# hila-chefer/Transformer-Explainability

Measured on AMD Instinct MI355X. Metric: relevance maps/sec (ViT-B/16 224^2, batch 64 per GPU, generate_LRP transformer_attribution), higher is better.
Workload: dtype f32 (3xbf16 split operands, 6 products, fp32 accumulate)

## Files before the change

### include/te_relprop.h

```cpp
#ifndef TE_RELPROP_H
#define TE_RELPROP_H

#include <stddef.h>
#include <stdint.h>

#ifdef __cplusplus
extern "C" {
#endif

typedef void* te_stream_t;
typedef uint16_t te_bf16_t;

enum {
  TE_OK = 0,
  TE_ERR_INVALID_ARG = -1,
  TE_ERR_WORKSPACE = -2,
  TE_ERR_UNSUPPORTED = -3,
  TE_ERR_NO_DEVICE = -4
};

enum { TE_VARIANT_OURS = 0, TE_VARIANT_LRP = 1, TE_IMPL_SIMPLE = 0x100 };

enum { TE_ROLLOUT_NORMALISE = 1, TE_ROLLOUT_CLS_FIXUP = 2, TE_ROLLOUT_ROW0 = 4 };

// ... 109 lines not shown
int te_gradcam_headmean_f32(const float* grad, const float* cam, float* out,
                            int64_t B, int64_t H, int64_t N, te_stream_t stream);

size_t te_rollout_workspace_bytes(int64_t L, int64_t B, int64_t N);
size_t te_rollout_row0_workspace_bytes(int64_t B, int64_t N);
int te_rollout_f32(const float* cams, int64_t L, int64_t start_layer, int64_t B, int64_t N,
                   int flags, float* joint, void* ws, size_t ws_bytes, te_stream_t stream);

#define TE_X6_TILE_AUTO 0
#define TE_X6_TILE_128 1
#define TE_X6_TILE_256 2
#define TE_X6_TILE_128x128 3
#define TE_X6_TEST_DROP_HANDOVER 0x200
#define TE_X6_WHOLE_TILES 0x10000
#define TE_X6_TEST_SMALL_GRID 0x4000
#define TE_X6_TILE_Z_SHIFT 10
#define TE_X6_TILE_C_SHIFT 12
#define TE_X6_PHASE_SPLIT 4
#define TE_X6_PHASE_Z 8
#define TE_X6_PHASE_C 16
#define TE_X6_PHASE_MASK 28
int te_linear_relprop_x6_supported(int64_t T, int64_t in_f, int64_t out_f);
size_t te_linear_relprop_x6_workspace_bytes(int64_t T, int64_t in_f, int64_t out_f);
size_t te_linear_x6_weight_planes_bytes(int64_t in_f, int64_t out_f);
size_t te_linear_x6_planes_bytes(int64_t rows, int64_t K);
int te_linear_x6_prepare_weights_f32(const float* W, int64_t in_f, int64_t out_f, void* planes, size_t planes_bytes,
                                     te_stream_t stream);
int te_linear_x6_split_abs_f32(const float* X, int64_t rows, int64_t K, void* planes, size_t planes_bytes,
                               te_stream_t stream);
int te_linear_relprop_x6_f32(const float* R, const float* r_scale, int64_t r_scale_stride, int64_t rows_per_sample,
// ... 301 lines not shown
```

### transformer-explainability_amd/csrc/te_api.hip

```cpp
#include "te_common.h"

#include <string.h>

extern "C" int te_version(void) { return 705;  }

#ifndef TE_BUILD_ID
#define TE_BUILD_ID "unstamped"
#endif
extern "C" const char* te_build_id(void) { return TE_BUILD_ID; }

extern "C" const char* te_status_string(int status) {
  switch (status) {
    case TE_OK: return "ok";
    case TE_ERR_INVALID_ARG: return "invalid argument";
    case TE_ERR_WORKSPACE: return "workspace missing, misaligned or too small";
    case TE_ERR_UNSUPPORTED: return "shape not supported by the gfx950 kernels";
    case TE_ERR_NO_DEVICE: return "no gfx950 device visible";
    default: break;
  }
  if (status > 0) return hipGetErrorString((hipError_t)status);
  return "unknown status";
}

extern "C" int te_device_check(void) {
// ... 10 lines not shown
```

### transformer-explainability_amd/csrc/te_linear_x6.hip

```cpp
#include <algorithm>
#include <cmath>
#include <type_traits>

#include "te_x6.h"

namespace {

constexpr int kRB = 3 * kFrag;
constexpr int kMinFrag = 4;
constexpr float kCancelTol = 0.0078125f;
constexpr int kSpinMillis = 250;
constexpr int kErrWord = 1023;


enum { MODE_Z = 0, MODE_C = 1, MODE_G = 2, MODE_ZI = 3, MODE_Z1 = 4, MODE_CI = 5, MODE_X = 6 };

__device__ __forceinline__ float bf16_f32(unsigned b) { return __uint_as_float(b << 16); }

enum { OP_ABS = 0, OP_POS = 1, OP_NEG = 2, OP_ID = 3 };
template <int OP>
__device__ __forceinline__ float apply_op(float x) {
  if constexpr (OP == OP_ID) return x;
  if constexpr (OP == OP_ABS) return __int_as_float(__float_as_int(x) & 0x7fffffff);
  const int b = __float_as_int(x);
  if constexpr (OP == OP_POS) return __int_as_float(b > 0 ? b : 0);
  return __int_as_float(b < 0 ? b : 0);
}

template <int OP, bool TRANSPOSE>
__global__ __launch_bounds__(256) void split_kernel(const float* __restrict__ src, unsigned char* __restrict__ dst,
// ... 104 lines not shown
  unsigned p[8][3];
#pragma unroll
  for (int e = 0; e < 8; ++e) split3_pk(v[2 * e], v[2 * e + 1], p[e]);
  auto store = [&](unsigned char* d) __attribute__((always_inline)) {
#pragma unroll
    for (int q = 0; q < 3; ++q)
#pragma unroll
      for (int kh = 0; kh < 2; ++kh) {
        u32x4 w;
#pragma unroll
        for (int e = 0; e < 4; ++e) w[e] = p[4 * kh + e][q];
        *reinterpret_cast<u32x4*>(d + q * kFrag + kh * 512) = w;
      }
  };
  store(dst + ((rb * nks + ks) * 3) * kFrag + r * 16);
  if constexpr (SRC == SRC_GELU_FWD) {
#pragma unroll
    for (int e = 0; e < 8; ++e) {
      const unsigned m = p[e][0] & 0x80008000u;
      p[e][0] &= 0x7fff7fffu;
      p[e][1] ^= m & (((p[e][1] & 0x7fff7fffu) + 0x7fff7fffu) & 0x80008000u);
      p[e][2] ^= m & (((p[e][2] & 0x7fff7fffu) + 0x7fff7fffu) & 0x80008000u);
    }
    store(dst_abs + ((rb * nks + ks) * 3) * kFrag + r * 16);
  }
}

__global__ __launch_bounds__(256) void zero_words_kernel(u32x4* __restrict__ p) {
  p[(size_t)blockIdx.x * 256 + threadIdx.x] = u32x4{0u, 0u, 0u, 0u};
}

// ... 67 lines not shown

constexpr int kStages = 2;
template <int WM>
struct X6Geo {
  static constexpr int NWM = (WM == 1) ? 1 : 2, NWN = (WM == 0) ? 2 : 4, MI = (WM == 0) ? 2 : 4;
  static constexpr int NW = NWM * NWN, THREADS = 64 * NW, WPS = (WM == 0) ? 3 : 2;
  static constexpr int TM = NWM * MI * 32, TT = NWN * 64;
  static constexpr int NPA = 3 * NWM * MI, NPB = 3 * NWN * 2;
  static constexpr int ACC = MI * 2 * 16;
  static constexpr int MAX_SPX = (WM == 2) ? 32 : (WM == 1) ? 64 : 96;
};

template <int WM, int MODE>
struct X6Lds {
  using GEO = X6Geo<WM>;
  static constexpr bool STAGED = (MODE == MODE_Z || MODE == MODE_ZI || MODE == MODE_Z1) && GEO::MI == 4;
  static constexpr int STAGES = kStages * (GEO::NPA + GEO::NPB) * kFrag;
  static constexpr int MAIN = (STAGED && GEO::NW * 16384 > STAGES) ? GEO::NW * 16384 : STAGES;
  static constexpr int TOTAL = MAIN + GEO::NW * 512 + 16;
};

template <int WM, int MODE>
__global__ __launch_bounds__(X6Geo<WM>::THREADS, X6Geo<WM>::WPS) void x6_kernel(const X6Params p) {
  using GEO = X6Geo<WM>;
  constexpr int NW = GEO::NW, NWM = GEO::NWM, NWN = GEO::NWN, MI = GEO::MI;
  constexpr bool IS_Z = (MODE == MODE_Z || MODE == MODE_ZI || MODE == MODE_Z1);
  constexpr bool IS_C = (MODE == MODE_C || MODE == MODE_CI);
  constexpr int G = IS_C ? 6 : 3;
  constexpr int NPA = GEO::NPA, NPB = GEO::NPB;
  constexpr int NP = NPA + NPB;
  static_assert(NPA / 3 == NW, "each wave stages one weight-side block");
  constexpr int PBW = NPB / 3 / NW;
  constexpr int STAGE = NP * kFrag;
  constexpr int GROUPS = NPA / G;
  constexpr int LDS_MAIN = X6Lds<WM, MODE>::MAIN;
  extern __shared__ __attribute__((aligned(16))) unsigned char smem[];

  const int lane = threadIdx.x & 63;
  const int wave = __builtin_amdgcn_readfirstlane(threadIdx.x >> 6);
  const int wm = wave / NWN, wn = wave % NWN;
  const int lane16 = lane * 16;
// ... 43 lines not shown
    }

    const unsigned char* srcA;
    if constexpr (!IS_C)
      srcA = p.A + (int64_t)(tm * GROUPS + wave) * p.a_group_stride + (int64_t)k0 * kRB;
    else
      srcA = p.A + (int64_t)(tm * GROUPS + (wave >> 1)) * p.a_group_stride + (int64_t)k0 * (2 * kRB) + (wave & 1) * kRB;
    const unsigned char* srcB[PBW];
#pragma unroll
    for (int u = 0; u < PBW; ++u) {
      const int cb = min(tn * (GEO::TT / 32) + wave * PBW + u, p.ncb - 1);
      srcB[u] = p.B + (int64_t)cb * p.b_rb_stride + (int64_t)k0 * kRB;
    }
    unsigned char* const ldsA = smem + wave * kRB;
    unsigned char* const ldsB = smem + NPA * kFrag + wave * (PBW * kRB);
    auto stage_in = [&](int stg, int adv) __attribute__((always_inline)) {
      srcA += adv * (G * kFrag);
#pragma unroll
      for (int u = 0; u < PBW; ++u) srcB[u] += adv * kRB;
#pragma unroll
      for (int q = 0; q < 3; ++q) glds16(srcA + q * kFrag + lane16, ldsA + stg * STAGE + q * kFrag);
#pragma unroll
      for (int u = 0; u < PBW; ++u)
#pragma unroll
        for (int q = 0; q < 3; ++q) glds16(srcB[u] + q * kFrag + lane16, ldsB + stg * STAGE + (u * 3 + q) * kFrag);
    };

    auto wait_for = [&](unsigned* flag) -> bool {
      unsigned* const ok_word = reinterpret_cast<unsigned*>(smem + LDS_MAIN + NW * 512);
      if (threadIdx.x == 0) {
        unsigned spins = 0, ok = 1u;
        const long long t_begin = wall_clock64();
        while (__hip_atomic_load(flag, __ATOMIC_RELAXED, __HIP_MEMORY_SCOPE_AGENT) == 0u) {
          __builtin_amdgcn_s_sleep(8);
          if ((++spins & 63u) == 0u &&
              (__hip_atomic_load(p.status, __ATOMIC_RELAXED, __HIP_MEMORY_SCOPE_AGENT) != 0u ||
               wall_clock64() - t_begin > p.spin_ticks)) {
            ok = 0u;
            break;
          }
// ... 24 lines not shown
            for (int e = 0; e < 4; ++e) acc[mi][ni][4 * c + e] = handed_over ? v[e] : __builtin_nanf("");
          }
          ip += 4 * 64;
          asm volatile("" : "+v"(ip));
        }
    } else {
#pragma unroll
      for (int mi = 0; mi < MI; ++mi)
#pragma unroll
        for (int ni = 0; ni < 2; ++ni)
#pragma unroll
          for (int e = 0; e < 16; ++e) acc[mi][ni][e] = 0.0f;
    }

    stage_in(0, 0);
    int st = 0;
    bf16x8 a[MI][3], b[2][3];
    for (int ks = k0; ks < k1; ++ks) {
      asm volatile("s_waitcnt vmcnt(0) lgkmcnt(0)" ::: "memory");
      __builtin_amdgcn_s_barrier();
      const unsigned char* sA = smem + st * STAGE + wm * (MI * kRB) + lane16;
      const unsigned char* sB = smem + st * STAGE + NPA * kFrag + wn * (2 * kRB) + lane16;
      const unsigned aA = (unsigned)(uintptr_t)sA, aB = (unsigned)(uintptr_t)sB;
#define X6_SB __builtin_amdgcn_sched_barrier(0)
#define X6_RDB(ni, r) \
  asm volatile("ds_read_b128 %0, %1 offset:%2" : "=v"(b[ni][PB[r]]) : "v"(aB), "i"((ni) * kRB + PB[r] * kFrag))
#define X6_RDA(mi, r) \
  asm volatile("ds_read_b128 %0, %1 offset:%2" : "=v"(a[mi][PA[r]]) : "v"(aA), "i"((mi) * kRB + PA[r] * kFrag))
#define X6_WAIT(n)                                                           \
  X6_SB;                                                                     \
// ... 50 lines not shown
      X6_SB;
#pragma unroll
      for (int q6 = 3; q6 < 6; ++q6) {
        X6_MM(0, 0, q6); X6_MM(1, 0, q6); X6_MM(1, 1, q6); X6_MM(0, 1, q6);
        X6_MM(2, 1, q6); X6_MM(2, 0, q6); X6_MM(3, 0, q6); X6_MM(3, 1, q6);
        X6_SB;
      }
      }
#undef X6_SB
#undef X6_RDB
#undef X6_RDA
#undef X6_WAIT
#undef X6_MM
#undef X6_RD_HEAD
#undef X6_RD_TAIL
      st = (st + 1 == kStages) ? 0 : st + 1;
    }

    auto publish = [&](float* dst, unsigned* flag) __attribute__((always_inline)) {
      f32x4* op = reinterpret_cast<f32x4*>(dst) + (size_t)wave * (GEO::ACC / 4) * 64 + lane;
#pragma unroll
      for (int mi = 0; mi < MI; ++mi)
#pragma unroll
        for (int ni = 0; ni < 2; ++ni) {
#pragma unroll
          for (int c = 0; c < 4; ++c) {
            f32x4 v;
#pragma unroll
            for (int e = 0; e < 4; ++e) v[e] = acc[mi][ni][4 * c + e];
            op[c * 64] = v;
          }
          op += 4 * 64;
// ... 73 lines not shown
          for (int g = 0; g < 4; ++g) {
            asm volatile("ds_read_b128 %0, %1 offset:%2" : "=v"(r4[g]) : "v"(rda[g]), "i"(buf * 8192));
            if constexpr (MODE != MODE_Z1)
              asm volatile("ds_read_b128 %0, %1 offset:%2" : "=v"(y4[g]) : "v"(rda[g]), "i"(buf * 8192 + 4096));
            asm volatile("ds_read_b128 %0, %1 offset:%2" : "=v"(b4[g]) : "v"(bia), "i"((mi * 32 + 8 * g) * 4));
          }
          asm volatile("s_waitcnt lgkmcnt(0)" ::: "memory");
          if (bi + 2 < 2 * MI) request(bi + 2, buf);
          X6_PASS4(r4[0], r4[1], r4[2], r4[3]);
          if constexpr (MODE != MODE_Z1) X6_PASS4(y4[0], y4[1], y4[2], y4[3]);
          X6_PASS4(b4[0], b4[1], b4[2], b4[3]);
          unsigned w[4][3][2];
          unsigned long long any_cancel = 0;
          auto z_of = [&](int g, int c0, f32x2& z2, f32x2& a2) __attribute__((always_inline)) {
            a2 = f32x2{acc[mi][ni][4 * g + c0], acc[mi][ni][4 * g + c0 + 1]};
            if constexpr (MODE == MODE_Z)
              z2 = f32x2{0.5f, 0.5f} * ((f32x2{y4[g][c0], y4[g][c0 + 1]} - f32x2{b4[g][c0], b4[g][c0 + 1]}) + a2);
            else if constexpr (MODE == MODE_ZI)
              z2 = f32x2{0.5f, 0.5f} * ((f32x2{y4[g][c0], y4[g][c0 + 1]} - f32x2{b4[g][c0], b4[g][c0 + 1]}) - a2);
            else
              z2 = a2;
          };
          auto cancels = [&](float z, float a_abs) __attribute__((always_inline)) -> bool {
            if constexpr (MODE == MODE_Z) return !(z > kCancelTol * a_abs);
            else if constexpr (MODE == MODE_ZI) return !(-z > kCancelTol * a_abs);
            else return false;
          };
#pragma unroll
          for (int g = 0; g < 4; ++g) {
            float sv4[4];
#pragma unroll
            for (int c0 = 0; c0 < 4; c0 += 2) {
              f32x2 z2, a2;
              z_of(g, c0, z2, a2);
              f32x2 rr = {r4[g][c0], r4[g][c0 + 1]};
              if (p.rs) rr = rr * f32x2{f[ni], f[ni]};
              const f32x2 sv = sd2(rr, z2);
#pragma unroll
              for (int e = 0; e < 2; ++e) {
// ... 87 lines not shown
          if (bi + 1 < 2 * MI) load_block(bi + 1, buf ^ 1);
        } else {
          load_block(bi, 0);
        }
        unsigned w[4][3][2];
        unsigned bad = 0;
#pragma unroll
        for (int g = 0; g < 4; ++g) {
          const f32x4 b4 = *reinterpret_cast<const f32x4*>(bias_lds + mi * 32 + 8 * g + 4 * h);
          float sv4[4];
#pragma unroll
          for (int c = 0; c < 4; ++c) {
            const float a_abs = acc[mi][ni][4 * g + c];
            float z;
            bool cancel;
            if constexpr (MODE == MODE_Z) {
              z = 0.5f * ((y4[buf][g][c] - b4[c]) + a_abs);
              cancel = !(z > kCancelTol * a_abs);
            } else if constexpr (MODE == MODE_ZI) {
              z = 0.5f * ((y4[buf][g][c] - b4[c]) - a_abs);
              cancel = !(-z > kCancelTol * a_abs);
            } else {
              z = a_abs;
              cancel = false;
            }
            bad |= (cancel ? 1u : 0u) << (4 * g + c);
            float rr = r4[buf][g][c];
            if (p.rs) rr = rr * f[ni];
            float sv = te_sd(rr, z);
            asm volatile("" : "+v"(sv));
            sv4[c] = (live[ni] && !cancel) ? sv : 0.0f;
// ... 180 lines not shown
inline X6Workspace general_workspace(int64_t T, int64_t in_f, int64_t out_f) { return x6_workspace(T, in_f, out_f, 2, 2, kGeneralPasses); }

struct X6WeightPlanes { size_t c, total; };
inline X6WeightPlanes weight_planes(int64_t in_f, int64_t out_f) {
  const size_t c = te_align_up(planes_bytes(out_f, in_f), 256);
  return {c, c + te_align_up(2 * planes_bytes(in_f, out_f), 256)};
}
struct X6WeightPlanesLrp { size_t wn, wpT, wnT, total; };
inline X6WeightPlanesLrp weight_planes_lrp(int64_t in_f, int64_t out_f) {
  const size_t za = te_align_up(planes_bytes(out_f, in_f), 256), ca = te_align_up(planes_bytes(in_f, out_f), 256);
  return {za, 2 * za, 2 * za + ca, 2 * za + 2 * ca};
}

constexpr int kTileMask = TE_X6_TILE_128 | TE_X6_TILE_256 | TE_X6_TILE_128x128;
constexpr int kProductFlags = kTileMask | TE_X6_WHOLE_TILES | TE_X6_TEST_DROP_HANDOVER | TE_X6_TEST_SMALL_GRID;
constexpr int kRuleFlags = kProductFlags | TE_X6_PHASE_MASK | (kTileMask << TE_X6_TILE_Z_SHIFT) | (kTileMask << TE_X6_TILE_C_SHIFT);

inline int pick_wm(int64_t in_f, int64_t out_f) {
  if (out_f % 256 == 0 && in_f % 128 == 0) return 2;
  if (out_f % 128 == 0 && in_f % 64 == 0) return 1;
  return 0;
}

inline long long spin_ticks_for_current_device() {
  static long long cached[64] = {};
  int dev = 0;
  if (hipGetDevice(&dev) != hipSuccess || dev < 0 || dev >= 64) dev = 0;
  if (cached[dev] == 0) {
    int khz = 0;
    if (hipDeviceGetAttribute(&khz, hipDeviceAttributeWallClockRate, dev) != hipSuccess || khz <= 0) khz = 100000;
    cached[dev] = (long long)khz * kSpinMillis;
// ... 166 lines not shown
  return TE_OK;
}

extern "C" int te_gelu_backward_x6_planes_f32(const float* dy, const float* x, int64_t rows, int64_t K, void* planes,
                                              size_t planes_bytes_, te_stream_t stream_) {
  const int rc = check_producer(dy && x && planes, te_aligned16(dy) && te_aligned16(x), te_aligned16(planes), rows, K, planes_bytes_);
  if (rc != TE_OK) return rc;
  gelu_split_lds_kernel<SRC_GELU_BWD><<<producer_grid(rows, K), dim3(256), 0, (hipStream_t)stream_>>>(
      dy, x, nullptr, (unsigned char*)planes, nullptr, rows, K);
  TE_RETURN_IF_LAUNCH_FAILED();
  return TE_OK;
}

extern "C" int te_gelu_forward_x6_planes_f32(const float* x, float* y, int64_t rows, int64_t K, void* planes, void* planes_abs,
                                             size_t planes_bytes_, te_stream_t stream_) {
  const int rc = check_producer(x && y && planes && planes_abs, te_aligned16(x) && te_aligned16(y),
                                te_aligned16(planes) && te_aligned16(planes_abs), rows, K, planes_bytes_);
  if (rc != TE_OK) return rc;
  gelu_split_lds_kernel<SRC_GELU_FWD><<<producer_grid(rows, K), dim3(256), 0, (hipStream_t)stream_>>>(
      nullptr, x, y, (unsigned char*)planes, (unsigned char*)planes_abs, rows, K);
  TE_RETURN_IF_LAUNCH_FAILED();
  return TE_OK;
}

extern "C" size_t te_gemm_x6_workspace_bytes(int64_t T, int64_t K, int64_t M) {
  return te_gemm_x6_supported(T, K, M) ? gemm_workspace(T, K, M).total : 0;
}

extern "C" int te_gemm_x6_f32(const float* X, const void* x_planes, const void* w_planes, const float* bias, float* out,
                              int64_t T, int64_t K, int64_t M, int flags, unsigned* status, void* ws, size_t ws_bytes,
                              te_stream_t stream_) {
  if ((!X && !x_planes) || !w_planes || !out) return TE_ERR_INVALID_ARG;
// ... 32 lines not shown
  if (!te_linear_relprop_x6_supported(T, in_f, out_f)) return TE_ERR_UNSUPPORTED;
  if (!ws || ws_bytes < te_linear_relprop_x6_workspace_bytes(T, in_f, out_f) || !te_aligned16(ws)) return TE_ERR_WORKSPACE;
  if (!te_aligned16(X) || !te_aligned16(W) || !te_aligned16(R) || !te_aligned16(Y) || !te_aligned16(out) ||
      !te_aligned16(w_planes) || (bias && !te_aligned16(bias)) || (x_planes && !te_aligned16(x_planes)))
    return TE_ERR_UNSUPPORTED;
  if (bad_r_scale(r_scale, rows_per_sample, T)) return TE_ERR_INVALID_ARG;
  if ((flags & ~kRuleFlags) != 0) return TE_ERR_INVALID_ARG;
  const int phases = (flags & TE_X6_PHASE_MASK) ? (flags & TE_X6_PHASE_MASK) : TE_X6_PHASE_MASK;
  hipStream_t stream = (hipStream_t)stream_;
  const X6Workspace l = rule_workspace(T, in_f, out_f);
  unsigned char* Ss = l.sp(ws, 0);
  const unsigned char* wz = (const unsigned char*)w_planes;
  const unsigned char* wc = wz + weight_planes(in_f, out_f).c;

  if (phases & TE_X6_PHASE_SPLIT) zero_flag_regions(l.flag_region(ws, 0), kRulePasses, stream);
  if (!x_planes) {
    if (phases & TE_X6_PHASE_SPLIT) {
      int rc = te_linear_x6_split_abs_f32(X, T, in_f, l.x(ws, 0), planes_bytes(T, in_f), stream_);
      if (rc != TE_OK) return rc;
    }
    x_planes = l.x(ws, 0);
  }
  const int wm_max = pick_wm(in_f, out_f);
  const int pz = (flags >> TE_X6_TILE_Z_SHIFT) & kTileMask, pc = (flags >> TE_X6_TILE_C_SHIFT) & kTileMask;
  const int wm_z = choose_geo(wm_max, T, out_f, pz ? pz : (flags & kTileMask), 256, true);
  const int wm_c = choose_geo(wm_max, T, 2 * in_f, pc ? pc : (flags & kTileMask));
  const X6Params p = rule_params(call_params(T, l.acc(ws), bias, out, status, flags), R, r_scale, r_scale_stride, rows_per_sample,
                                 X, W, Y);
  int rc;
  if (phases & TE_X6_PHASE_Z) {
    rc = launch_pass<MODE_Z>(p, wm_z, wz, (const unsigned char*)x_planes, Ss, in_f, out_f, l.flag_region(ws, 0), stream, 1.0f);
    if (rc != TE_OK) return rc;
  }
  if (phases & TE_X6_PHASE_C) {
    rc = launch_pass<MODE_C>(p, wm_c, wc, Ss, Ss, in_f, out_f, l.flag_region(ws, 1), stream, 1.0f);
    if (rc != TE_OK) return rc;
  }
  TE_RETURN_IF_LAUNCH_FAILED();
  return TE_OK;
}

extern "C" int te_linear_relprop_x6_general_supported(int64_t T, int64_t in_f, int64_t out_f, int variant) {
  if (!te_linear_relprop_x6_supported(T, in_f, out_f)) return 0;
  if (variant == TE_VARIANT_LRP) return (in_f % 128 == 0) ? 1 : 0;
  return variant == TE_VARIANT_OURS ? 1 : 0;
}
// ... 123 lines not shown
```

### transformer-explainability_amd/ops.py

```python
from __future__ import annotations

import contextlib
import os
from typing import Optional, Sequence, Tuple

import torch

from . import _lib
from ._lib import (TE_HEADMEAN_CLAMP, TE_HEADMEAN_ROW0, TE_IMPL_SIMPLE, TE_RATIONALE_CLAMP, TE_ROLLOUT_CLS_FIXUP,
                   TE_ROLLOUT_NORMALISE, TE_ROLLOUT_ROW0, TE_VARIANT_LRP, TE_VARIANT_OURS)
from ._lib import (TE_X6_PHASE_C, TE_X6_PHASE_SPLIT, TE_X6_PHASE_Z, TE_X6_TEST_DROP_HANDOVER,
                   TE_X6_TEST_SMALL_GRID, TE_X6_TILE_C_SHIFT, TE_X6_TILE_Z_SHIFT, TE_X6_WHOLE_TILES)

Tensor = torch.Tensor
_VARIANTS = {"ours": TE_VARIANT_OURS, "lrp": TE_VARIANT_LRP}

FORCE_SIMPLE = False
KERNEL_TIMER = None
_NULL = contextlib.nullcontext()


def _timed(name: str, flops: float = 0.0, nbytes: float = 0.0):
    return _NULL if KERNEL_TIMER is None else KERNEL_TIMER(name, float(flops), float(nbytes))


class Deferred:
    __slots__ = ("t", "scale")
# ... 265 lines not shown
    out_f, in_f = W.shape
    dims = (in_f, out_f) if transposed else (out_f, in_f)
    return _cached_planes(W, cache, "x6_gemm_planes_T" if transposed else "x6_gemm_planes", lambda Wd: (_prepare_planes(
        _c(Wd), "te_linear_x6_planes_bytes", "te_linear_x6_split_matrix_f32", dims, int(transposed)),))[0]


def linear_relprop_x6_supported(T: int, in_f: int, out_f: int) -> bool:
    return bool(_lib.load().te_linear_relprop_x6_supported(int(T), int(in_f), int(out_f)))


def gemm_x6_supported(T: int, K: int, M: int) -> bool:
    return bool(_lib.load().te_gemm_x6_supported(int(T), int(K), int(M)))


X6_KEEP_ABS = os.environ.get("TE_X6_KEEP_ABS", "1") not in ("", "0")


def _x_abs_key(X: Tensor, T: int, K: int):
    return (X.data_ptr(), X._version, T, K, str(X.device))


def post_x_planes(cache: dict, X: Tensor, xs: Tensor, xa: Tensor):
    K = X.shape[-1]
    cache["x_planes_from_producer"] = (_x_abs_key(X, X.numel() // K, K), xs, xa, X)


def take_x_planes(cache: dict, X: Tensor, T: int, K: int):
    hit = cache.pop("x_planes_from_producer", None)
    if hit is not None and hit[0] == _x_abs_key(X, T, K) and hit[3].data_ptr() == X.data_ptr():
        return hit[1], hit[2]
    return None


def drop_x_planes(cache: dict, with_abs: bool = False):
    cache.pop("x_planes_from_producer", None)
    if with_abs:
        cache.pop("x_abs_planes", None)
# ... 52 lines not shown
    K = X.shape[-1]
    lead = X.shape[:-1]
    T = X.numel() // K
    Xc = None if x_planes is not None else _c(X).reshape(-1, K)
    like = X if Xc is None else Xc
    out = torch.empty((T, M), dtype=torch.float32, device=X.device)
    bc = None if bias is None else _c(bias.detach())
    with _on_device(like) as lib:
        ws = _ws(lib.te_gemm_x6_workspace_bytes(T, K, M), like)
        x_bytes = (6.0 if x_planes is not None else 10.0) * T * K
        xs = x_planes
        if xs is None and keep_abs is not None:
            got = take_x_planes(keep_abs, X, T, K)
            if got is not None:
                xs, x_bytes = got[0], 6.0 * T * K
                post_x_abs_planes(keep_abs, X, T, K, got[1])
        if xs is not None and xs.numel() * xs.element_size() < lib.te_linear_x6_planes_bytes(T, K):
            raise _lib.TeError(f"gemm_x6: the operand planes handed in hold {xs.numel() * xs.element_size()} bytes, "
                               f"[{T}, {K}] needs {lib.te_linear_x6_planes_bytes(T, K)}")
        with _timed(timer_name, 12.0 * T * K * M, x_bytes + 6.0 * K * M + 4.0 * T * M):
            if xs is None and keep_abs is not None and rule_takes_abs_planes(T, K, M):
                nb = lib.te_linear_x6_planes_bytes(T, K)
                xs, xa = _ws(nb, Xc), _ws(nb, Xc)
                _lib.check(lib.te_linear_x6_split_dual_f32(_ptr(Xc), T, K, _ptr(xs), _ptr(xa), nb, _stream(Xc)),
                           "te_linear_x6_split_dual_f32")
                post_x_abs_planes(keep_abs, X, T, K, xa)
            _lib.check(lib.te_gemm_x6_f32(_ptr(Xc) if Xc is not None else None, _ptr(xs), _ptr(w_planes), _ptr(bc), _ptr(out),
                                          T, K, M, (X6_TILE | X6_FLAGS) & ~0x3c00, _ptr(x6_status(X.device)), _ptr(ws),
                                          ws.numel(), _stream(like)), "te_gemm_x6_f32")
    return out.reshape(*lead, M)


def linear_relprop(R: Tensor, X: Tensor, W: Tensor, alpha: float = 1.0, variant="ours",
                   Y: Optional[Tensor] = None, bias: Optional[Tensor] = None, cache: Optional[dict] = None) -> Tensor:
    if _any_f64(R, X, W):
        return linear_relprop_f64(R, X, W, alpha=alpha, variant=variant)
    if _is_bf16(X) or _is_bf16(W):
        return linear_relprop_bf16(R, X, W, alpha=alpha, variant=variant, cache=cache)
    out_f, in_f = W.shape
    lead = X.shape[:-1]
    R, r_scale = _split_deferred(R)
# ... 15 lines not shown
    var_code = var & 0xff
    general = (USE_LINEAR_X6 and not (var & TE_IMPL_SIMPLE) and not (var_code == TE_VARIANT_OURS and alpha == 1)
               and all(t.data_ptr() % 16 == 0 for t in (Rc, Xc, Wc))
               and (var_code == TE_VARIANT_LRP or (USE_FORWARD_OUTPUT and Y is not None))
               and bool(_lib.load().te_linear_relprop_x6_general_supported(T, in_f, out_f, var_code)))
    if general:
        Yg = bg = None
        if var_code == TE_VARIANT_OURS:
            Yg = _c(Y.detach()).reshape(-1, out_f)
            bg = None if bias is None else _c(bias.detach())
            general = Yg.shape[0] == T and Yg.data_ptr() % 16 == 0 and (bg is None or bg.data_ptr() % 16 == 0)
    if general:
        wp = x6_weight_planes(W, cache) if var_code == TE_VARIANT_OURS else None
        wpl = x6_weight_planes_lrp(W, cache) if var_code == TE_VARIANT_LRP else None
        xa = take_x_abs_planes(cache, X, T, in_f) if cache is not None and var_code == TE_VARIANT_OURS else None
        gemm = 2.0 * T * in_f * out_f
        halves = 2 if alpha != 1 else 1
        units = (18.0 if var_code == TE_VARIANT_OURS else 24.0) * halves
        with _on_device(Xc) as lib, _timed("linear_x6_general", units * gemm,
                                           halves * (6.0 * (2 * T * in_f + 3 * in_f * out_f + 2 * T * out_f) + 16.0 * T * in_f)):
            ws = _ws(lib.te_linear_relprop_x6_general_workspace_bytes(T, in_f, out_f, var_code), Xc)
            _lib.check(lib.te_linear_relprop_x6_general_f32(_ptr(Rc), rs_ptr, rs_stride, rps, _ptr(Xc), _ptr(Wc), _ptr(wp),
                                                            _ptr(wpl), _ptr(xa), _ptr(Yg), _ptr(bg), _ptr(out), T, in_f,
                                                            out_f, float(alpha), var_code, (X6_TILE | X6_FLAGS) & ~0x3c00,
                                                            _ptr(x6_status(Xc.device)), _ptr(ws), ws.numel(), _stream(Xc)),
                       "te_linear_relprop_x6_general_f32")
            if X6_CHECK:
                x6_raise_if_failed(Xc.device)
        return out.reshape(*lead, in_f)
    if fwd:
        Yc = _c(Y.detach()).reshape(-1, out_f)
        bc = None if bias is None else _c(bias.detach())
        if Yc.shape[0] != T:
            raise _lib.TeError(f"Linear.relprop: Y has {Yc.shape[0]} rows, X has {T}")
    if (fwd and USE_LINEAR_X6 and Yc.data_ptr() % 16 == 0 and (bc is None or bc.data_ptr() % 16 == 0)
            and _lib.load().te_linear_relprop_x6_supported(T, in_f, out_f)):
        planes = x6_weight_planes(W, cache)
        xa = take_x_abs_planes(cache, X, T, in_f) if cache is not None else None
        with _on_device(Xc) as lib:
            ws = _ws(lib.te_linear_relprop_x6_workspace_bytes(T, in_f, out_f), Xc)
            status = x6_status(Xc.device)

            def call(flags):
                _lib.check(lib.te_linear_relprop_x6_f32(_ptr(Rc), rs_ptr, rs_stride, rps, _ptr(Xc), _ptr(Wc), _ptr(planes),
                                                        _ptr(xa), _ptr(Yc), _ptr(bc), _ptr(out), T, in_f, out_f,
                                                        X6_TILE | X6_FLAGS | flags, _ptr(status), _ptr(ws), ws.numel(),
                                                        _stream(Xc)),
                           "te_linear_relprop_x6_f32")
            if KERNEL_TIMER is None:
                call(0)
            else:
                gemm = 2.0 * T * in_f * out_f
                if xa is None:
                    with _timed("linear_x6_split", 0.0, 10.0 * T * in_f):
                        call(TE_X6_PHASE_SPLIT)
                else:
                    call(TE_X6_PHASE_SPLIT)
                with _timed("linear_x6_zpass", 6.0 * gemm, 6.0 * (T * in_f + in_f * out_f + T * out_f) + 8.0 * T * out_f):
                    call(TE_X6_PHASE_Z)
                with _timed("linear_x6_cpass", 12.0 * gemm, 6.0 * (T * out_f + 2 * in_f * out_f) + 8.0 * T * in_f):
                    call(TE_X6_PHASE_C)
# ... 242 lines not shown
        _lib.check(lib.te_attention_backward_strided_f32(_ptr(d_out), N * C, 64, C, _ptr(q), qb, qh, qn, _ptr(k), kb, kh, kn,
                                                         _ptr(v), vb, vh, vn, _ptr(attn), _ptr(d_attn), _ptr(dq), dqb, dqh,
                                                         dqn, _ptr(dk), dkb, dkh, dkn, _ptr(dv), dvb, dvh, dvn, B, H, N, D,
                                                         float(scale), int(bool(need_qk)), _ptr(ws), ws.numel(),
                                                         _stream(d_out)), "te_attention_backward_strided_f32")
    return d_attn


def attention_forward_planes_supported(qkv: Tensor, num_heads: int) -> bool:
    B, N, C3 = qkv.shape
    C = C3 // 3
    return (qkv.is_cuda and qkv.dtype == torch.float32 and C % num_heads == 0 and C // num_heads == 64 and N <= 224
            and bool(_lib.load().te_attention_forward_supported(N, 64)))


def attention_forward(qkv: Tensor, num_heads: int, scale: float, planes: bool = False):
    if _is_bf16(qkv):
        if planes:
            raise _lib.TeError("attention_forward(planes=True): operand planes are emitted from float32 activations only")
        qkv = _c16(qkv)
        C = qkv.shape[-1] // 3
        out, attn, zqk, _ = attention_forward_qkv_bf16(qkv[..., :C], qkv[..., C:2 * C], qkv[..., 2 * C:], num_heads, scale)
        return out, attn, zqk
    qkv = _c(qkv)
    B, N, C3 = qkv.shape
    C = C3 // 3
    H, D = num_heads, C // num_heads
    if not _lib.load().te_attention_forward_supported(N, D):
        if planes:
            raise _lib.TeError("attention_forward(planes=True): shape not served by te_attention_forward_planes_f32")
        out, attn, zqk, _ = attention_forward_qkv(qkv[..., :C], qkv[..., C:2 * C], qkv[..., 2 * C:], num_heads, scale)
        return out, attn, zqk
    out = torch.empty((B, N, C), dtype=torch.float32, device=qkv.device)
    attn = torch.empty((B, H, N, N), dtype=torch.float32, device=qkv.device)
    zqk = torch.empty((B, H, N, N), dtype=torch.float32, device=qkv.device)
    extra = 12.0 * B * N * C if planes else 0.0
    with _on_device(qkv) as lib, _timed("attention_forward", 4.0 * B * H * N * N * D, 4.0 * B * (2 * H * N * N + 4 * N * C) + extra):
        if planes:
            nb = lib.te_linear_x6_planes_bytes(B * N, C)
            xs, xa = _ws(nb, qkv), _ws(nb, qkv)
            _lib.check(lib.te_attention_forward_planes_f32(_ptr(qkv), _ptr(zqk), _ptr(attn), _ptr(out), _ptr(xs), _ptr(xa), nb,
                                                           B, H, N, D, float(scale), _stream(qkv)),
                       "te_attention_forward_planes_f32")
            return out, attn, zqk, xs, xa
        _lib.check(lib.te_attention_forward_f32(_ptr(qkv), _ptr(zqk), _ptr(attn), _ptr(out), B, H, N, D, float(scale),
                                                _stream(qkv)), "te_attention_forward_f32")
    return out, attn, zqk


def attention_backward(d_out: Tensor, qkv: Tensor, attn: Tensor, num_heads: int, scale: float,
                       need_qk: bool = True, out: Optional[Tensor] = None) -> Tuple[Tensor, Optional[Tensor]]:
    if _is_bf16(d_out) or _is_bf16(qkv) or _is_bf16(attn):
        qkv = _c16(qkv)
        C = qkv.shape[-1] // 3
        d_qkv = torch.empty_like(qkv)
# ... 79 lines not shown
        return self

    def __exit__(self, *exc):
        global _GELU_BWD_HANDOFF
        _GELU_BWD_HANDOFF -= 1


def gelu_backward_handoff_active() -> bool:
    return _GELU_BWD_HANDOFF > 0


def gelu_planes_supported(x: Tensor) -> bool:
    return bool(X6_FUSE_GELU and x.dim() >= 2 and x.shape[-1] >= 16 and x.shape[-1] % 16 == 0)


def gelu_forward_planes(x: Tensor):
    x = _c(x)
    K = x.shape[-1]
    T = x.numel() // K
    y = torch.empty_like(x)
    with _on_device(x) as lib, _timed("gelu_forward", 0.0, (4.0 * 2 + 12.0) * x.numel()):
        nb = lib.te_linear_x6_planes_bytes(T, K)
        xs, xa = _ws(nb, x), _ws(nb, x)
        _lib.check(lib.te_gelu_forward_x6_planes_f32(_ptr(x), _ptr(y), T, K, _ptr(xs), _ptr(xa), nb, _stream(x)),
                   "te_gelu_forward_x6_planes_f32")
    return y, xs, xa


def gelu_backward_planes(dy: Tensor, x: Tensor) -> Tensor:
    dy, x = _c(dy), _c(x)
    K = x.shape[-1]
    T = x.numel() // K
    with _on_device(x) as lib, _timed("gelu_backward", 0.0, (4.0 * 2 + 6.0) * x.numel()):
        nb = lib.te_linear_x6_planes_bytes(T, K)
        planes = _ws(nb, x)
        _lib.check(lib.te_gelu_backward_x6_planes_f32(_ptr(dy), _ptr(x), T, K, _ptr(planes), nb, _stream(x)),
                   "te_gelu_backward_x6_planes_f32")
    return planes
# ... 1313 lines not shown
```

### transformer-explainability_amd/producers.py

```python
from __future__ import annotations

import torch

from . import ops


def usable(x: torch.Tensor) -> bool:
    return ops.USE_FUSED_PRODUCERS and torch.is_tensor(x) and ops.layernorm_supported(x)


def gelu_usable(x: torch.Tensor) -> bool:
    return (ops.USE_FUSED_PRODUCERS and torch.is_tensor(x) and x.is_cuda and x.dtype == torch.float32
            and x.numel() > 0 and x.numel() % 4 == 0)


def norm_usable(x: torch.Tensor, norm) -> bool:
    return (usable(x) and not norm.training and getattr(norm, "weight", None) is not None
            and tuple(norm.normalized_shape) == (x.shape[-1],))


class _LayerNorm(torch.autograd.Function):
    @staticmethod
    def forward(ctx, x, weight, bias, eps):
        y, mean, rstd = ops.layernorm_forward(x, weight, bias, eps)
# ... 17 lines not shown
    @staticmethod
    def backward(ctx, d_bypass, dy):
        x, weight, mean, rstd = ctx.saved_tensors
        if dy is None:
            return d_bypass, None, None, None
        return ops.layernorm_backward(dy, x, weight, mean, rstd, add=d_bypass), None, None, None


class _Gelu(torch.autograd.Function):

    @staticmethod
    def forward(ctx, x, feeds, source):
        ctx.save_for_backward(x)
        ctx.source = source
        if feeds is not None:
            y, xs, xa = ops.gelu_forward_planes(x)
            ops.post_x_planes(feeds, y, xs, xa)
            return y
        return ops.gelu_forward(x)

    @staticmethod
    def backward(ctx, dy):
        (x,) = ctx.saved_tensors
        if ctx.source is not None:
            return ops.post_dy_planes(ctx.source, ops.gelu_backward_planes(dy, x), x), None, None
        return ops.gelu_backward(dy, x), None, None


class _Linear(torch.autograd.Function):

    @staticmethod
# ... 64 lines not shown
```

### transformer-explainability_amd/vit.py

```python
from __future__ import annotations

import torch
import torch.nn as nn

from . import methods, ops, producers
from . import rules as R_ours

__all__ = ["VisionTransformer", "vit_base_patch16_224", "vit_large_patch16_224", "deit_base_patch16_224",
           "compute_rollout_attention", "make_vit_module"]


def compute_rollout_attention(all_layer_matrices, start_layer=0):
    return ops.rollout(torch.stack(list(all_layer_matrices), 0), start_layer=start_layer, normalise=False)


def tail_full(model, cam, **kwargs):
    cam, _ = model.add.relprop(cam, **kwargs)
    cam = model.patch_embed.relprop(cam[:, 1:], **kwargs)
    return cam.sum(dim=1)


def tail_rollout(model, start_layer=0):
    mats = [blk.attn.get_attn_cam().clamp(min=0).mean(dim=1) for blk in model.blocks]
    return compute_rollout_attention(mats, start_layer=start_layer)[:, 0, 1:]
# ... 62 lines not shown
                slot.zero_()
            else:
                slot.copy_(g)
        return grad.view(B, N, 3 * H * D), None


def split_qkv(qkv, num_heads):
    return _SplitQKV.apply(qkv, num_heads)


class _FusedAttention(torch.autograd.Function):

    @staticmethod
    def forward(ctx, qkv, num_heads, scale, module, feeds=None):
        if feeds is not None:
            out, attn, zqk, xs, xa = ops.attention_forward(qkv, num_heads, scale, planes=True)
            ops.post_x_planes(feeds, out, xs, xa)
        else:
            out, attn, zqk = ops.attention_forward(qkv, num_heads, scale)
        ctx.save_for_backward(qkv, attn, out)
        ctx.num_heads, ctx.scale, ctx.module = num_heads, scale, module
        ctx.mark_non_differentiable(attn, zqk)
        ctx.set_materialize_grads(False)
        return out, attn, zqk

    @staticmethod
    def backward(ctx, d_out, _d_attn_unused, _d_zqk_unused):
        qkv, attn, out = ctx.saved_tensors
        if d_out is None:
            return None, None, None, None, None
        stop = bool(getattr(ctx.module, "_fused_stop_backward", False))
# ... 363 lines not shown
```

Measured before the change: 1012.

## Reuse signed operand planes for relprop Z pass by taking abs on the fly

Producers (GELU, attention, forward GEMM split) no longer write a second set of absolute-value bf16 planes. The Z relevance pass gets a new signed mode that loads the signed X planes into registers, clears the sign of the high plane, flips the lower planes to match, and stores them to LDS itself instead of using direct global-to-LDS loads. This saves the extra plane writes and their memory footprint in the forward pass. In exchange the Z kernel does more register and ALU work and loses the asynchronous LDS load path, which could hurt its pipelining.

```diff
diff --git a/include/te_relprop.h b/include/te_relprop.h
--- a/include/te_relprop.h
+++ b/include/te_relprop.h
@@ -147,6 +147,7 @@
 #define TE_X6_TEST_DROP_HANDOVER 0x200
 #define TE_X6_WHOLE_TILES 0x10000
 #define TE_X6_TEST_SMALL_GRID 0x4000
+#define TE_X6_X_PLANES_SIGNED 0x20000
 #define TE_X6_TILE_Z_SHIFT 10
 #define TE_X6_TILE_C_SHIFT 12
 #define TE_X6_PHASE_SPLIT 4
diff --git a/transformer-explainability_amd/csrc/te_api.hip b/transformer-explainability_amd/csrc/te_api.hip
--- a/transformer-explainability_amd/csrc/te_api.hip
+++ b/transformer-explainability_amd/csrc/te_api.hip
@@ -2,7 +2,7 @@
 
 #include <string.h>
 
-extern "C" int te_version(void) { return 705;  }
+extern "C" int te_version(void) { return 706;  }
 
 #ifndef TE_BUILD_ID
 #define TE_BUILD_ID "unstamped"
diff --git a/transformer-explainability_amd/csrc/te_linear_x6.hip b/transformer-explainability_amd/csrc/te_linear_x6.hip
--- a/transformer-explainability_amd/csrc/te_linear_x6.hip
+++ b/transformer-explainability_amd/csrc/te_linear_x6.hip
@@ -13,7 +13,7 @@
 constexpr int kErrWord = 1023;
 
 
-enum { MODE_Z = 0, MODE_C = 1, MODE_G = 2, MODE_ZI = 3, MODE_Z1 = 4, MODE_CI = 5, MODE_X = 6 };
+enum { MODE_Z = 0, MODE_C = 1, MODE_G = 2, MODE_ZI = 3, MODE_Z1 = 4, MODE_CI = 5, MODE_X = 6, MODE_ZS = 7 };
 
 __device__ __forceinline__ float bf16_f32(unsigned b) { return __uint_as_float(b << 16); }
 
@@ -148,7 +148,7 @@
       }
   };
   store(dst + ((rb * nks + ks) * 3) * kFrag + r * 16);
-  if constexpr (SRC == SRC_GELU_FWD) {
+  if (SRC == SRC_GELU_FWD && dst_abs) {
 #pragma unroll
     for (int e = 0; e < 8; ++e) {
       const unsigned m = p[e][0] & 0x80008000u;
@@ -246,7 +246,7 @@
 template <int WM, int MODE>
 struct X6Lds {
   using GEO = X6Geo<WM>;
-  static constexpr bool STAGED = (MODE == MODE_Z || MODE == MODE_ZI || MODE == MODE_Z1) && GEO::MI == 4;
+  static constexpr bool STAGED = (MODE == MODE_Z || MODE == MODE_ZS || MODE == MODE_ZI || MODE == MODE_Z1) && GEO::MI == 4;
   static constexpr int STAGES = kStages * (GEO::NPA + GEO::NPB) * kFrag;
   static constexpr int MAIN = (STAGED && GEO::NW * 16384 > STAGES) ? GEO::NW * 16384 : STAGES;
   static constexpr int TOTAL = MAIN + GEO::NW * 512 + 16;
@@ -256,7 +256,9 @@
 __global__ __launch_bounds__(X6Geo<WM>::THREADS, X6Geo<WM>::WPS) void x6_kernel(const X6Params p) {
   using GEO = X6Geo<WM>;
   constexpr int NW = GEO::NW, NWM = GEO::NWM, NWN = GEO::NWN, MI = GEO::MI;
-  constexpr bool IS_Z = (MODE == MODE_Z || MODE == MODE_ZI || MODE == MODE_Z1);
+  constexpr bool SGN = MODE == MODE_ZS;
+  constexpr bool Z_ABS = MODE == MODE_Z || SGN;
+  constexpr bool IS_Z = (Z_ABS || MODE == MODE_ZI || MODE == MODE_Z1);
   constexpr bool IS_C = (MODE == MODE_C || MODE == MODE_CI);
   constexpr int G = IS_C ? 6 : 3;
   constexpr int NPA = GEO::NPA, NPB = GEO::NPB;
@@ -330,6 +332,7 @@
     }
     unsigned char* const ldsA = smem + wave * kRB;
     unsigned char* const ldsB = smem + NPA * kFrag + wave * (PBW * kRB);
+    u32x4 breg[SGN ? PBW : 1][3];
     auto stage_in = [&](int stg, int adv) __attribute__((always_inline)) {
       srcA += adv * (G * kFrag);
 #pragma unroll
@@ -339,7 +342,24 @@
 #pragma unroll
       for (int u = 0; u < PBW; ++u)
 #pragma unroll
-        for (int q = 0; q < 3; ++q) glds16(srcB[u] + q * kFrag + lane16, ldsB + stg * STAGE + (u * 3 + q) * kFrag);
+        for (int q = 0; q < 3; ++q) {
+          if constexpr (SGN) breg[u][q] = *reinterpret_cast<const u32x4*>(srcB[u] + q * kFrag + lane16);
+          else glds16(srcB[u] + q * kFrag + lane16, ldsB + stg * STAGE + (u * 3 + q) * kFrag);
+        }
+    };
+    auto sign_and_store = [&](int stg) __attribute__((always_inline)) {
+#pragma unroll
+      for (int u = 0; u < (SGN ? PBW : 0); ++u) {
+#pragma unroll
+        for (int e = 0; e < 4; ++e) {
+          const unsigned m = breg[u][0][e] & 0x80008000u;
+          breg[u][0][e] &= 0x7fff7fffu;
+          breg[u][1][e] ^= m;
+          breg[u][2][e] ^= m;
+        }
+#pragma unroll
+        for (int q = 0; q < 3; ++q) *reinterpret_cast<u32x4*>(ldsB + stg * STAGE + (u * 3 + q) * kFrag + lane16) = breg[u][q];
+      }
     };
 
     auto wait_for = [&](unsigned* flag) -> bool {
@@ -394,6 +414,7 @@
     }
 
     stage_in(0, 0);
+    if constexpr (SGN) sign_and_store(0);
     int st = 0;
     bf16x8 a[MI][3], b[2][3];
     for (int ks = k0; ks < k1; ++ks) {
@@ -474,8 +495,10 @@
 #undef X6_MM
 #undef X6_RD_HEAD
 #undef X6_RD_TAIL
+      if constexpr (SGN) sign_and_store((st + 1) % kStages);
       st = (st + 1 == kStages) ? 0 : st + 1;
     }
+    if constexpr (SGN) asm volatile("s_waitcnt lgkmcnt(0)" ::: "memory");
 
     auto publish = [&](float* dst, unsigned* flag) __attribute__((always_inline)) {
       f32x4* op = reinterpret_cast<f32x4*>(dst) + (size_t)wave * (GEO::ACC / 4) * 64 + lane;
@@ -579,7 +602,7 @@
           unsigned long long any_cancel = 0;
           auto z_of = [&](int g, int c0, f32x2& z2, f32x2& a2) __attribute__((always_inline)) {
             a2 = f32x2{acc[mi][ni][4 * g + c0], acc[mi][ni][4 * g + c0 + 1]};
-            if constexpr (MODE == MODE_Z)
+            if constexpr (Z_ABS)
               z2 = f32x2{0.5f, 0.5f} * ((f32x2{y4[g][c0], y4[g][c0 + 1]} - f32x2{b4[g][c0], b4[g][c0 + 1]}) + a2);
             else if constexpr (MODE == MODE_ZI)
               z2 = f32x2{0.5f, 0.5f} * ((f32x2{y4[g][c0], y4[g][c0 + 1]} - f32x2{b4[g][c0], b4[g][c0 + 1]}) - a2);
@@ -587,7 +610,7 @@
               z2 = a2;
           };
           auto cancels = [&](float z, float a_abs) __attribute__((always_inline)) -> bool {
-            if constexpr (MODE == MODE_Z) return !(z > kCancelTol * a_abs);
+            if constexpr (Z_ABS) return !(z > kCancelTol * a_abs);
             else if constexpr (MODE == MODE_ZI) return !(-z > kCancelTol * a_abs);
             else return false;
           };
@@ -705,7 +728,7 @@
             const float a_abs = acc[mi][ni][4 * g + c];
             float z;
             bool cancel;
-            if constexpr (MODE == MODE_Z) {
+            if constexpr (Z_ABS) {
               z = 0.5f * ((y4[buf][g][c] - b4[c]) + a_abs);
               cancel = !(z > kCancelTol * a_abs);
             } else if constexpr (MODE == MODE_ZI) {
@@ -916,7 +939,7 @@
 
 constexpr int kTileMask = TE_X6_TILE_128 | TE_X6_TILE_256 | TE_X6_TILE_128x128;
 constexpr int kProductFlags = kTileMask | TE_X6_WHOLE_TILES | TE_X6_TEST_DROP_HANDOVER | TE_X6_TEST_SMALL_GRID;
-constexpr int kRuleFlags = kProductFlags | TE_X6_PHASE_MASK | (kTileMask << TE_X6_TILE_Z_SHIFT) | (kTileMask << TE_X6_TILE_C_SHIFT);
+constexpr int kRuleFlags = kProductFlags | TE_X6_PHASE_MASK | TE_X6_X_PLANES_SIGNED | (kTileMask << TE_X6_TILE_Z_SHIFT) | (kTileMask << TE_X6_TILE_C_SHIFT);
 
 inline int pick_wm(int64_t in_f, int64_t out_f) {
   if (out_f % 256 == 0 && in_f % 128 == 0) return 2;
@@ -1113,8 +1136,8 @@
 
 extern "C" int te_gelu_forward_x6_planes_f32(const float* x, float* y, int64_t rows, int64_t K, void* planes, void* planes_abs,
                                              size_t planes_bytes_, te_stream_t stream_) {
-  const int rc = check_producer(x && y && planes && planes_abs, te_aligned16(x) && te_aligned16(y),
-                                te_aligned16(planes) && te_aligned16(planes_abs), rows, K, planes_bytes_);
+  const int rc = check_producer(x && y && planes, te_aligned16(x) && te_aligned16(y),
+                                te_aligned16(planes) && (!planes_abs || te_aligned16(planes_abs)), rows, K, planes_bytes_);
   if (rc != TE_OK) return rc;
   gelu_split_lds_kernel<SRC_GELU_FWD><<<producer_grid(rows, K), dim3(256), 0, (hipStream_t)stream_>>>(
       nullptr, x, y, (unsigned char*)planes, (unsigned char*)planes_abs, rows, K);
@@ -1177,9 +1200,11 @@
   const unsigned char* wc = wz + weight_planes(in_f, out_f).c;
 
   if (phases & TE_X6_PHASE_SPLIT) zero_flag_regions(l.flag_region(ws, 0), kRulePasses, stream);
+  const bool x_signed = (flags & TE_X6_X_PLANES_SIGNED) != 0;
   if (!x_planes) {
     if (phases & TE_X6_PHASE_SPLIT) {
-      int rc = te_linear_x6_split_abs_f32(X, T, in_f, l.x(ws, 0), planes_bytes(T, in_f), stream_);
+      int rc = x_signed ? te_linear_x6_split_matrix_f32(X, T, in_f, 0, l.x(ws, 0), planes_bytes(T, in_f), stream_)
+                        : te_linear_x6_split_abs_f32(X, T, in_f, l.x(ws, 0), planes_bytes(T, in_f), stream_);
       if (rc != TE_OK) return rc;
     }
     x_planes = l.x(ws, 0);
@@ -1192,7 +1217,8 @@
                                  X, W, Y);
   int rc;
   if (phases & TE_X6_PHASE_Z) {
-    rc = launch_pass<MODE_Z>(p, wm_z, wz, (const unsigned char*)x_planes, Ss, in_f, out_f, l.flag_region(ws, 0), stream, 1.0f);
+    rc = x_signed ? launch_pass<MODE_ZS>(p, wm_z, wz, (const unsigned char*)x_planes, Ss, in_f, out_f, l.flag_region(ws, 0), stream, 1.0f)
+                  : launch_pass<MODE_Z>(p, wm_z, wz, (const unsigned char*)x_planes, Ss, in_f, out_f, l.flag_region(ws, 0), stream, 1.0f);
     if (rc != TE_OK) return rc;
   }
   if (phases & TE_X6_PHASE_C) {
diff --git a/transformer-explainability_amd/ops.py b/transformer-explainability_amd/ops.py
--- a/transformer-explainability_amd/ops.py
+++ b/transformer-explainability_amd/ops.py
@@ -10,7 +10,7 @@
 from ._lib import (TE_HEADMEAN_CLAMP, TE_HEADMEAN_ROW0, TE_IMPL_SIMPLE, TE_RATIONALE_CLAMP, TE_ROLLOUT_CLS_FIXUP,
                    TE_ROLLOUT_NORMALISE, TE_ROLLOUT_ROW0, TE_VARIANT_LRP, TE_VARIANT_OURS)
 from ._lib import (TE_X6_PHASE_C, TE_X6_PHASE_SPLIT, TE_X6_PHASE_Z, TE_X6_TEST_DROP_HANDOVER,
-                   TE_X6_TEST_SMALL_GRID, TE_X6_TILE_C_SHIFT, TE_X6_TILE_Z_SHIFT, TE_X6_WHOLE_TILES)
+                   TE_X6_TEST_SMALL_GRID, TE_X6_TILE_C_SHIFT, TE_X6_TILE_Z_SHIFT, TE_X6_WHOLE_TILES, TE_X6_X_PLANES_SIGNED)
 
 Tensor = torch.Tensor
 _VARIANTS = {"ours": TE_VARIANT_OURS, "lrp": TE_VARIANT_LRP}
@@ -306,13 +306,23 @@
 
 
 X6_KEEP_ABS = os.environ.get("TE_X6_KEEP_ABS", "1") not in ("", "0")
+X6_SIGNED_PLANES = True
+
+
+def _signed(planes: Tensor) -> Tensor:
+    planes._te_signed_planes = True
+    return planes
+
+
+def planes_are_signed(planes: Optional[Tensor]) -> bool:
+    return planes is not None and getattr(planes, "_te_signed_planes", False)
 
 
 def _x_abs_key(X: Tensor, T: int, K: int):
     return (X.data_ptr(), X._version, T, K, str(X.device))
 
 
-def post_x_planes(cache: dict, X: Tensor, xs: Tensor, xa: Tensor):
+def post_x_planes(cache: dict, X: Tensor, xs: Tensor, xa: Optional[Tensor] = None):
     K = X.shape[-1]
     cache["x_planes_from_producer"] = (_x_abs_key(X, X.numel() // K, K), xs, xa, X)
 
@@ -395,17 +405,26 @@
             got = take_x_planes(keep_abs, X, T, K)
             if got is not None:
                 xs, x_bytes = got[0], 6.0 * T * K
-                post_x_abs_planes(keep_abs, X, T, K, got[1])
+                post_x_abs_planes(keep_abs, X, T, K, got[1] if got[1] is not None else _signed(xs))
         if xs is not None and xs.numel() * xs.element_size() < lib.te_linear_x6_planes_bytes(T, K):
             raise _lib.TeError(f"gemm_x6: the operand planes handed in hold {xs.numel() * xs.element_size()} bytes, "
                                f"[{T}, {K}] needs {lib.te_linear_x6_planes_bytes(T, K)}")
+        for_rule = xs is None and keep_abs is not None and rule_takes_abs_planes(T, K, M)
+        if for_rule and not X6_SIGNED_PLANES:
+            x_bytes += 6.0 * T * K
         with _timed(timer_name, 12.0 * T * K * M, x_bytes + 6.0 * K * M + 4.0 * T * M):
-            if xs is None and keep_abs is not None and rule_takes_abs_planes(T, K, M):
+            if for_rule:
                 nb = lib.te_linear_x6_planes_bytes(T, K)
-                xs, xa = _ws(nb, Xc), _ws(nb, Xc)
-                _lib.check(lib.te_linear_x6_split_dual_f32(_ptr(Xc), T, K, _ptr(xs), _ptr(xa), nb, _stream(Xc)),
-                           "te_linear_x6_split_dual_f32")
-                post_x_abs_planes(keep_abs, X, T, K, xa)
+                if X6_SIGNED_PLANES:
+                    xs = _signed(_ws(nb, Xc))
+                    _lib.check(lib.te_linear_x6_split_matrix_f32(_ptr(Xc), T, K, 0, _ptr(xs), nb, _stream(Xc)),
+                               "te_linear_x6_split_matrix_f32")
+                    post_x_abs_planes(keep_abs, X, T, K, xs)
+                else:
+                    xs, xa = _ws(nb, Xc), _ws(nb, Xc)
+                    _lib.check(lib.te_linear_x6_split_dual_f32(_ptr(Xc), T, K, _ptr(xs), _ptr(xa), nb, _stream(Xc)),
+                               "te_linear_x6_split_dual_f32")
+                    post_x_abs_planes(keep_abs, X, T, K, xa)
             _lib.check(lib.te_gemm_x6_f32(_ptr(Xc) if Xc is not None else None, _ptr(xs), _ptr(w_planes), _ptr(bc), _ptr(out),
                                           T, K, M, (X6_TILE | X6_FLAGS) & ~0x3c00, _ptr(x6_status(X.device)), _ptr(ws),
                                           ws.numel(), _stream(like)), "te_gemm_x6_f32")
@@ -451,6 +470,8 @@
         wp = x6_weight_planes(W, cache) if var_code == TE_VARIANT_OURS else None
         wpl = x6_weight_planes_lrp(W, cache) if var_code == TE_VARIANT_LRP else None
         xa = take_x_abs_planes(cache, X, T, in_f) if cache is not None and var_code == TE_VARIANT_OURS else None
+        if planes_are_signed(xa):
+            xa = None
         gemm = 2.0 * T * in_f * out_f
         halves = 2 if alpha != 1 else 1
         units = (18.0 if var_code == TE_VARIANT_OURS else 24.0) * halves
@@ -474,6 +495,7 @@
             and _lib.load().te_linear_relprop_x6_supported(T, in_f, out_f)):
         planes = x6_weight_planes(W, cache)
         xa = take_x_abs_planes(cache, X, T, in_f) if cache is not None else None
+        x_signed = TE_X6_X_PLANES_SIGNED if planes_are_signed(xa) else 0
         with _on_device(Xc) as lib:
             ws = _ws(lib.te_linear_relprop_x6_workspace_bytes(T, in_f, out_f), Xc)
             status = x6_status(Xc.device)
@@ -481,7 +503,7 @@
             def call(flags):
                 _lib.check(lib.te_linear_relprop_x6_f32(_ptr(Rc), rs_ptr, rs_stride, rps, _ptr(Xc), _ptr(Wc), _ptr(planes),
                                                         _ptr(xa), _ptr(Yc), _ptr(bc), _ptr(out), T, in_f, out_f,
-                                                        X6_TILE | X6_FLAGS | flags, _ptr(status), _ptr(ws), ws.numel(),
+                                                        X6_TILE | X6_FLAGS | x_signed | flags, _ptr(status), _ptr(ws), ws.numel(),
                                                         _stream(Xc)),
                            "te_linear_relprop_x6_f32")
             if KERNEL_TIMER is None:
@@ -754,7 +776,7 @@
             and bool(_lib.load().te_attention_forward_supported(N, 64)))
 
 
-def attention_forward(qkv: Tensor, num_heads: int, scale: float, planes: bool = False):
+def attention_forward(qkv: Tensor, num_heads: int, scale: float, planes: bool = False, planes_abs: bool = True):
     if _is_bf16(qkv):
         if planes:
             raise _lib.TeError("attention_forward(planes=True): operand planes are emitted from float32 activations only")
@@ -774,11 +796,11 @@
     out = torch.empty((B, N, C), dtype=torch.float32, device=qkv.device)
     attn = torch.empty((B, H, N, N), dtype=torch.float32, device=qkv.device)
     zqk = torch.empty((B, H, N, N), dtype=torch.float32, device=qkv.device)
-    extra = 12.0 * B * N * C if planes else 0.0
+    extra = (12.0 if planes_abs else 6.0) * B * N * C if planes else 0.0
     with _on_device(qkv) as lib, _timed("attention_forward", 4.0 * B * H * N * N * D, 4.0 * B * (2 * H * N * N + 4 * N * C) + extra):
         if planes:
             nb = lib.te_linear_x6_planes_bytes(B * N, C)
-            xs, xa = _ws(nb, qkv), _ws(nb, qkv)
+            xs, xa = _ws(nb, qkv), _ws(nb, qkv) if planes_abs else None
             _lib.check(lib.te_attention_forward_planes_f32(_ptr(qkv), _ptr(zqk), _ptr(attn), _ptr(out), _ptr(xs), _ptr(xa), nb,
                                                            B, H, N, D, float(scale), _stream(qkv)),
                        "te_attention_forward_planes_f32")
@@ -888,14 +910,14 @@
     return bool(X6_FUSE_GELU and x.dim() >= 2 and x.shape[-1] >= 16 and x.shape[-1] % 16 == 0)
 
 
-def gelu_forward_planes(x: Tensor):
+def gelu_forward_planes(x: Tensor, planes_abs: bool = True):
     x = _c(x)
     K = x.shape[-1]
     T = x.numel() // K
     y = torch.empty_like(x)
-    with _on_device(x) as lib, _timed("gelu_forward", 0.0, (4.0 * 2 + 12.0) * x.numel()):
+    with _on_device(x) as lib, _timed("gelu_forward", 0.0, (4.0 * 2 + (12.0 if planes_abs else 6.0)) * x.numel()):
         nb = lib.te_linear_x6_planes_bytes(T, K)
-        xs, xa = _ws(nb, x), _ws(nb, x)
+        xs, xa = _ws(nb, x), _ws(nb, x) if planes_abs else None
         _lib.check(lib.te_gelu_forward_x6_planes_f32(_ptr(x), _ptr(y), T, K, _ptr(xs), _ptr(xa), nb, _stream(x)),
                    "te_gelu_forward_x6_planes_f32")
     return y, xs, xa
diff --git a/transformer-explainability_amd/producers.py b/transformer-explainability_amd/producers.py
--- a/transformer-explainability_amd/producers.py
+++ b/transformer-explainability_amd/producers.py
@@ -55,7 +55,7 @@
         ctx.save_for_backward(x)
         ctx.source = source
         if feeds is not None:
-            y, xs, xa = ops.gelu_forward_planes(x)
+            y, xs, xa = ops.gelu_forward_planes(x, not ops.X6_SIGNED_PLANES)
             ops.post_x_planes(feeds, y, xs, xa)
             return y
         return ops.gelu_forward(x)
diff --git a/transformer-explainability_amd/vit.py b/transformer-explainability_amd/vit.py
--- a/transformer-explainability_amd/vit.py
+++ b/transformer-explainability_amd/vit.py
@@ -100,7 +100,7 @@
     @staticmethod
     def forward(ctx, qkv, num_heads, scale, module, feeds=None):
         if feeds is not None:
-            out, attn, zqk, xs, xa = ops.attention_forward(qkv, num_heads, scale, planes=True)
+            out, attn, zqk, xs, xa = ops.attention_forward(qkv, num_heads, scale, planes=True, planes_abs=not ops.X6_SIGNED_PLANES)
             ops.post_x_planes(feeds, out, xs, xa)
         else:
             out, attn, zqk = ops.attention_forward(qkv, num_heads, scale)
```

Result: faster. 1024, median of 6 (+1.2%).
